# yellow-binary-tree/HeterSumGraph

Measured on AMD Instinct MI355X. Metric: graph-edges/sec through WSWGAT fwd+bwd, CNN/DM-shaped batch; 1/2/4/8 GPU, higher is better.
Workload: dtype f32; 1 GPU; cfg2: HSG WSWGAT stack W2S + 2x(S2W, W2S) fwd+bwd, train mode, 32 HSG docs/GPU x (N=35, W=600, k=36); gemm_operands=f32, bf16_rows=none, f32_rows=all, docs_per_gpu=32, graph_edges_per_gpu=159040, typed_edges_per_direction=40320, parallelism=dp1, dp_exchange=none (one rank), hip_graph=True

## Files before the change

### hetersumgraph_amd/_lib.py

```python
from __future__ import annotations

import ctypes
import os

import torch

_HERE = os.path.dirname(os.path.abspath(__file__))
LIB_PATH = os.environ.get("HSG_LIB_PATH") or os.path.join(_HERE, "libhsg.so")

HSG_EINVAL = 1001
HSG_TAU_TABLE = 0
HSG_TAU_PER_EDGE = 1

EXPORTS = ("hsg_gat_fwd", "hsg_gat_bwd_dst", "hsg_gat_bwd_blocks", "hsg_gat_bwd_src",
           "hsg_gat_bwd_src_blocks", "hsg_attn_src_logits", "hsg_attn_params_fwd", "hsg_attn_params_fwd_pair", "hsg_attn_params_fwd_pair_seed", "hsg_attn_params_finish_pair", "hsg_attn_params_bwd",
           "hsg_attn_params_bwd_workspace_floats", "hsg_version", "hsg_gemm_f32", "hsg_gemm_f32_mfma", "hsg_gemm_bf16", "hsg_gemm_workspace_floats", "hsg_gemm_auto_splits", "hsg_gemm_row_tiles", "hsg_ffn_colsums",
           "hsg_ln_bwd_blocks", "hsg_ln_fwd", "hsg_ln_bwd",
           "hsg_dropmask_words", "hsg_dropmask_scale", "hsg_dropmask", "hsg_hproj_fwd", "hsg_hproj_dx",
           "hsg_hproj_dw_chunks", "hsg_hproj_dw", "hsg_hproj_bwd", "hsg_rel_build_workspace_bytes", "hsg_rel_build",
           "hsg_cnn_taps", "hsg_cnn_gather", "hsg_cnn_pool", "hsg_cnn_pool_bwd",
           "hsg_ffn_small_supported", "hsg_ffn_small_fwd", "hsg_ffn_small_bwd_blocks", "hsg_ffn_small_bwd",
           "hsg_attn_params_stage", "hsg_attn_params_finish", "hsg_hproj_fwd_logits_supported",
           "hsg_hproj_fwd_logits", "hsg_wsplit_dims", "hsg_wsplit", "hsg_gemm_f32_psw", "hsg_dropmask_multi", "hsg_dropmask_multi_wt", "hsg_step_prologue", "hsg_gemm_f32_slabs", "hsg_slab_reduce",
           "hsg_hproj_wt", "hsg_hproj_fwd_t8_supported", "hsg_hproj_fwd_t8", "hsg_hproj_fwd_mf_supported", "hsg_hproj_fwd_mf", "hsg_kclock_arm",
           "hsg_kclock_pending", "hsg_seed_advance", "hsg_gat_bwd_dst_noh_supported", "hsg_gat_bwd_dst_noh",
           "hsg_gat_bwd_dst_g", "hsg_gemm_f32_psw_elug", "hsg_gemm_bf16_psw",
           "hsg_gemm_bf16_slabs", "hsg_gemm_dw_slabs", "hsg_gemm_dw_tiles", "hsg_gemm_psw_row_tiles", "hsg_gemm_psw_ln",
           "hsg_gat_bwd_src_g_supported", "hsg_gat_bwd_src_g", "hsg_gemm_psw_elug_rho", "hsg_ffn_small_bwd_gate",
           "hsg_gat_bwd_src_g_blocks", "hsg_gemm_bf16_psw_io", "hsg_gemm_bf16_psw_elug_rho_a16", "hsg_gemm_psw_elug_rho_gw", "hsg_ln_bwd_dy16",
           "hsg_gemm_dw_slabs_io", "hsg_ln_fwd_y16", "hsg_gat_bwd_src_g_io", "hsg_rel_work", "hsg_gat_fwd_ws_floats",
           "hsg_gat_fwd_ws", "hsg_gat_bwd_src_g_ws_floats", "hsg_gat_bwd_src_g_ws", "hsg_gat_fwd_ws16",
           "hsg_gemm_bf16_psw_elug_rho_x16", "hsg_ln_fwd_x16", "hsg_ln_bwd_x16")

HSG_EPI_STORE = 0
HSG_EPI_RELU_BWD = 1
HSG_EPI_ADD = 2
HSG_EPI_ADD_ELUG = 3
HSG_IO_A_BF16 = 1
HSG_IO_C_BF16 = 2
HSG_IO_AUX_BF16 = 4


class HsgRel(ctypes.Structure):

    _fields_ = [("n_src", ctypes.c_int32), ("n_dst", ctypes.c_int32), ("n_edges", ctypes.c_int32),
                ("indptr", ctypes.c_void_p), ("src", ctypes.c_void_p), ("tf", ctypes.c_void_p),
                ("phantom", ctypes.c_void_p), ("cindptr", ctypes.c_void_p),
                ("cdst", ctypes.c_void_p), ("cperm", ctypes.c_void_p),
                ("n_dwork", ctypes.c_int32), ("n_swork", ctypes.c_int32),
                ("dwork", ctypes.c_void_p), ("swork", ctypes.c_void_p)]


_lib = None

_P = ctypes.c_void_p
_I = ctypes.c_int
_F = ctypes.c_float
_RELP = ctypes.POINTER(HsgRel)

_SIGS = {
    "hsg_gat_fwd": [_RELP, _I, _I, _I, _F, _P, _P, _P, _P, _P, _P, _P, _P, _P],
    "hsg_gat_bwd_dst": [_RELP, _I, _I, _I, _I, _F, _P, _P, _P, _P, _P, _P, _P, _P, _P, _P, _P],
    "hsg_gat_bwd_blocks": [_RELP],
    "hsg_gat_bwd_src": [_RELP, _I, _I, _I, _F, _P, _P, _P, _P, _P, _P, _P, _P, _P, _P, _P, _P],
    "hsg_gat_bwd_src_blocks": [_RELP],
# ... 33 lines not shown
    "hsg_hproj_fwd_mf_supported": [_I, _I, _I],
    "hsg_hproj_fwd_mf": [_I, _I, _I, _P, _I, _P, _I, _I, _P, _F, _P, _I, _P, _P, _P],
    "hsg_hproj_dx": [_I, _I, _I, _I, _P, _I, _P, _P, _F, _P, _I, _I, _P],
    "hsg_hproj_dw_chunks": [_I, _I, _I, _I],
    "hsg_hproj_bwd": [_I, _I, _I, _I, _P, _I, _P, _P, _I, _P, _F, _P, _I, _I, _P, _P],
    "hsg_hproj_dw": [_I, _I, _I, _I, _P, _I, _P, _I, _P, _F, _P, _P, _I, _P],
    "hsg_rel_build_workspace_bytes": [_I, _I],
    "hsg_rel_build": [_F, _F, _I, _I] + [_P] * 17 + [ctypes.c_size_t, _P],
    "hsg_cnn_taps": [],
    "hsg_cnn_gather": [_I, _I, _I, _P, _P, _P, _P, ctypes.c_long, _P, _P],
    "hsg_cnn_pool": [_I, _I, _P, _P, _I, _P, _P, _P, _P],
    "hsg_cnn_pool_bwd": [_I, _P, _P, _P, _P, _P, _I, _P],
    "hsg_ln_fwd": [_I, _I, _P, _P, _P, _P, _F, _F, _P, ctypes.c_uint32, _P, _P, _P, _P],
    "hsg_ffn_small_supported": [_I, _I],
    "hsg_ffn_small_bwd_blocks": [_I],
    "hsg_ffn_small_bwd": [_I, _I, _I] + [_P] * 9 + [_F, _P, ctypes.c_uint32] + [_P] * 6,
    "hsg_ffn_small_bwd_gate": [_I, _I, _I] + [_P] * 9 + [_F, _P, ctypes.c_uint32] + [_P] * 9,
    "hsg_ffn_small_fwd": [_I, _I, _I, _P, _P, _P, _P, _P, _P, _P, _F, _F, _P, ctypes.c_uint32, _P, _P, _P, _P, _P,
                          _P],
    "hsg_ln_bwd": [_I, _I, _P, _P, _P, _P, _P, _P, _F, _P, ctypes.c_uint32, _P, _P, _P, _P],
    "hsg_wsplit_dims": [_I, _I, _P, _P],
    "hsg_dropmask_multi": [_I, _P, _P, _P, _P, _P, _P, _P, _P],
    "hsg_dropmask_multi_wt": [_I, _P, _P, _P, _P, _P, _P, _P, _I, _I, _I, _P, _P, _P],
    "hsg_step_prologue": [_I, _P, _P, _P, _P, _P, _P, _P, _I, _I, _I, _P, _P, _I, _P, _P, _P, _P, _P, _P, _P],
    "hsg_gemm_f32_slabs": [_I, _I, _I, _P, _I, _I, _P, _I, _I, _I, _P, _P],
    "hsg_gemm_bf16_slabs": [_I, _I, _I, _P, _I, _I, _P, _I, _I, _I, _P, _P],
    "hsg_gemm_dw_slabs": [_I, _P, _P, _I, _P, _P, _P, _P, _I, _I, _P, _P],
    "hsg_gemm_dw_tiles": [_I, _I],
    "hsg_gemm_psw_row_tiles": [_I, _I, _I, _I],
    "hsg_gemm_psw_ln": [_I, _I, _I, _P, _I, _P, _P, _P, _P, _P, _P, _F, _F, _P, ctypes.c_uint32, _P, _P, _P, _I, _P],
    "hsg_slab_reduce": [_I, _P, _P, _P, _P, _P, _P, _P, _P, _P, _P, _P],
    "hsg_wsplit": [_I, _P, _P, _P, _P, _P, _P, _P],
    "hsg_gemm_f32_psw": [_I, _I, _I, _P, _I, _P, _P, _I, _P, _P, _I, _I, _I, _P, _P],
    "hsg_gemm_f32_psw_elug": [_I, _I, _I, _P, _I, _P, _P, _I, _P, _P, _P, _P, _I, _I, _P],
    "hsg_gemm_bf16_psw": [_I, _I, _I, _P, _I, _P, _P, _I, _P, _P, _I, _I, _I, _P, _P],
    "hsg_gat_bwd_dst_g": [_RELP, _I, _I, _I, _F, _P, _P, _P, _P, _P, _P, _P, _P, _P],
    "hsg_gat_bwd_src_g_supported": [_RELP, _I, _I],
    "hsg_gat_bwd_src_g_blocks": [_RELP, _I, _I],
    "hsg_gat_bwd_src_g": [_RELP, _I, _I, _F, _P, _P, _P, _P, _P, _P, _I, _P, _P, _P, _P, _P, _P, _P],
    "hsg_gemm_psw_elug_rho": [_I, _I, _I, _P, _I, _P, _P, _I, _P, _P, _P, _P, _I, _P, _I, _I, _P],
    "hsg_gemm_bf16_psw_io": [_I, _I, _I, _P, _I, _P, _P, _I, _P, _P, _I, _I, _I, _P, _I, _P],
    "hsg_gemm_bf16_psw_elug_rho_a16": [_I, _I, _I, _P, _I, _P, _P, _I, _P, _P, _P, _P, _I, _P, _I, _I, _P],
    "hsg_gemm_psw_elug_rho_gw": [_I, _I, _I, _I, _I],
    "hsg_ln_bwd_dy16": [_I, _I, _P, _P, _I, _P, _P, _P, _P, _F, _P, ctypes.c_uint32, _P, _I, _P, _P, _P],
    "hsg_ln_fwd_y16": [_I, _I, _P, _P, _P, _P, _F, _F, _P, ctypes.c_uint32, _P, _P, _P, _P],
    "hsg_gat_bwd_src_g_io": [_RELP, _I, _I, _F, _P, _P, _P, _P, _P, _I, _P, _I, _P, _P, _P, _P, _P, _P, _P],
    "hsg_gemm_dw_slabs_io": [_I, _P, _P, _I, _P, _P, _P, _P, _P, _I, _P, _P],
    "hsg_rel_work": [_I, _P, _I, _I, _P, _I, _P, _P],
    "hsg_gat_fwd_ws_floats": [_RELP, _I, _I],
    "hsg_gat_fwd_ws": [_RELP, _I, _I, _I, _F, _P, _P, _P, _P, _P, _P, _P, _P, _P, _P],
    "hsg_gat_fwd_ws16": [_RELP, _I, _I, _I, _F, _P, _P, _P, _P, _P, _P, _P, _P, _P, _P, _I, _P],
    "hsg_gemm_bf16_psw_elug_rho_x16": [_I, _I, _I, _P, _I, _P, _P, _I, _P, _P, _I, _I, _P, _P, _I, _P, _I, _I, _P],
    "hsg_ln_fwd_x16": [_I, _I, _P, _P, _I, _P, _P, _F, _F, _P, ctypes.c_uint32, _P, _P, _P, _P],
    "hsg_ln_bwd_x16": [_I, _I, _P, _P, _P, _I, _P, _P, _P, _F, _P, ctypes.c_uint32, _P, _I, _P, _P, _P],
    "hsg_gat_bwd_src_g_ws_floats": [_RELP, _I, _I],
    "hsg_gat_bwd_src_g_ws": [_RELP, _I, _I, _F, _P, _P, _P, _P, _P, _I, _P, _I, _P, _P, _P, _P, _P, _P, _P, _P],
}
_RESTYPE = {"hsg_version": ctypes.c_char_p, "hsg_wsplit_dims": None, "hsg_gemm_workspace_floats": ctypes.c_size_t,
            "hsg_attn_params_bwd_workspace_floats": ctypes.c_size_t,
            "hsg_dropmask_scale": ctypes.c_float,
            "hsg_rel_build_workspace_bytes": ctypes.c_size_t, "hsg_gat_fwd_ws_floats": ctypes.c_size_t,
            "hsg_gat_bwd_src_g_ws_floats": ctypes.c_size_t}


def load():
    global _lib
# ... 108 lines not shown
```

### hetersumgraph_amd/csrc/hsg_gemm.hip

```cpp
#include <hip/hip_runtime.h>
#include <type_traits>
#include <stdint.h>
#include <stdlib.h>

#include <atomic>

#include "../../include/hsg.h"
#include "hsg_dev.h"
#include "hsg_wave.h"
#include "hsg_rng.h"
#include "hsg_wsplit.h"

namespace {

typedef float f32x16 __attribute__((ext_vector_type(16)));
typedef float f32x4 __attribute__((ext_vector_type(4)));
typedef __bf16 bf16x8 __attribute__((ext_vector_type(8)));

constexpr int kBK = 32;
constexpr int kPad = 4;

struct GemmArgs {
    int M, N, K;
    const float *A;
// ... 773 lines not shown
        bn = f32x4{0.f, 0.f, 0.f, 0.f};
        if (p.bias) bn = *reinterpret_cast<const f32x4 *>(p.bias + nc);
        if (p.epi != HSG_EPI_STORE) {
#pragma unroll
            for (int t = 0; t < STEPS; ++t) {
                const int m = min(row0 + min(t * RPS + rs, 31), p.M - 1);
                if constexpr (AUXBF) {
                    auxb[t] = *reinterpret_cast<const bf16x4v7 *>(
                        reinterpret_cast<const __bf16 *>(p.aux) + (size_t)m * p.ldaux + nc);
                } else {
                    aux[t] = *reinterpret_cast<const f32x4 *>(p.aux + (size_t)m * p.ldaux + nc);
                }
            }
        }
        if (p.epi == HSG_EPI_ADD_ELUG) {
#pragma unroll
            for (int t = 0; t < STEPS; ++t) {
                const int m = min(row0 + min(t * RPS + rs, 31), p.M - 1);
                const size_t o = (size_t)m * p.ldaux + nc;
                if constexpr (XBF) {
                    const bf16x4v7 xb = *reinterpret_cast<const bf16x4v7 *>(
                        reinterpret_cast<const __bf16 *>(p.aux2) + (size_t)m * p.ldx + nc);
                    ex[t] = f32x4{(float)xb[0], (float)xb[1], (float)xb[2], (float)xb[3]} -
                            *reinterpret_cast<const f32x4 *>(p.aux3 + o);
                } else {
                    ex[t] = *reinterpret_cast<const f32x4 *>(p.aux2 + o) - *reinterpret_cast<const f32x4 *>(p.aux3 + o);
                }
            }
        }
    }

    template <bool NS = false>
    __device__ __forceinline__ void finish(const float *wl, int row0, int col0, int lane, const GemmArgs &p,
                                           f32x4 &csum) {
        __builtin_amdgcn_s_waitcnt(0xc07f);
        __builtin_amdgcn_wave_barrier();
        const int q = lane % QS, rs = lane / QS;
        const int n = col0 + 4 * q;
        const bool qok = q < QPR && rs < RPS && n < p.N;
        const bool rho = p.epi == HSG_EPI_ADD_ELUG && p.rho;
        int slot[4] = {3, 3, 3, 3};
        if (rho) {
            const int hb = (n / GW * GW) / p.rho_d;
#pragma unroll
            for (int e = 0; e < 4; ++e) slot[e] = n + e < p.N ? (n + e) / p.rho_d - hb : 3;
        }
        csum = f32x4{0.f, 0.f, 0.f, 0.f};
#pragma unroll
        for (int t = 0; t < STEPS; ++t) {
            const int r = t * RPS + rs, m = row0 + r;
            const bool rok = r < 32 && m < p.M;
            float c[3] = {0.f, 0.f, 0.f};
            if (qok && rok) {
                f32x4 v = *reinterpret_cast<const f32x4 *>(&wl[r * LDW + 4 * q]);
                if (p.epi == HSG_EPI_RELU_BWD) {
                    if constexpr (AUXBF) {
#pragma unroll
                        for (int e = 0; e < 4; ++e) v[e] = (float)auxb[t][e] > 0.f ? v[e] : 0.f;
                    } else {
#pragma unroll
                        for (int e = 0; e < 4; ++e) v[e] = aux[t][e] > 0.f ? v[e] : 0.f;
                    }
                } else {
                    v += bn;
                    if (p.epi == HSG_EPI_ADD || p.epi == HSG_EPI_ADD_ELUG) v += aux[t];
                    if (p.relu) {
#pragma unroll
                        for (int e = 0; e < 4; ++e) v[e] = fmaxf(v[e], 0.f);
                    }
                }
                if constexpr (CBF) {
                    *reinterpret_cast<bf16x4v7 *>(reinterpret_cast<__bf16 *>(p.C) + (size_t)m * p.ldc + n) =
                        bf16x4v7{(__bf16)v[0], (__bf16)v[1], (__bf16)v[2], (__bf16)v[3]};
                } else if (!NS || v[0] == 1234.5f) {
                    *reinterpret_cast<f32x4 *>(p.C + (size_t)m * p.ldc + n) = v;
                }
                if (p.epi == HSG_EPI_ADD_ELUG) {
                    f32x4 g;
#pragma unroll
                    for (int e = 0; e < 4; ++e) g[e] = ex[t][e] > 0.f ? v[e] : v[e] * (ex[t][e] + 1.f);
                    if constexpr (GBF)
                        *reinterpret_cast<bf16x4v7 *>(reinterpret_cast<__bf16 *>(p.C2) + (size_t)m * p.ldaux + n) =
                            bf16x4v7{(__bf16)g[0], (__bf16)g[1], (__bf16)g[2], (__bf16)g[3]};
                    else
// ... 399 lines not shown
            }
        }
        __builtin_amdgcn_iglp_opt(0);
    }

    __syncthreads();
    float *wl = lds + wid * 32 * (BN + 4);
    const int c = lane & 15, rq = 4 * (lane >> 4);
#pragma unroll
    for (int i = 0; i < 2; ++i)
#pragma unroll
        for (int j = 0; j < TN; ++j)
#pragma unroll
            for (int e = 0; e < 4; ++e) wl[(16 * i + rq + e) * (BN + 4) + 16 * j + c] = acc[i][j][e];
    f32x4 cs;
    if (nt == 0) ep.load(p, m0 + wid * 32, n0, lane);
    ep.template finish<PM == 4>(wl, m0 + wid * 32, n0, lane, p, cs);
    if (p.colpart) epi_rows_colpart<BN>(lds, cs, wid, lane, ty, n0, p);
}

template <int BN, int S, int PM = 0, int OCC = 2, bool SA = false, int IO = 0>
int launch7(GemmArgs p, const __bf16 *planes, int Np, int Kp, hipStream_t st) {
    p.splits = 1;
    p.k_tiles_per_split = Kp / 32;
    if ((p.N + BN - 1) / BN * BN > Np) return HSG_EINVAL;
    if (!epi_rows_ok(p)) return HSG_EINVAL;
    const long g = (long)((p.N + BN - 1) / BN) * ((p.M + 127) / 128);
    if (SA && ((long)p.M * p.lda * 4 >= (1L << 32) || (long)3 * Np * Kp * 2 >= (1L << 32))) return HSG_EINVAL;
    hipLaunchKernelGGL((k_gemm7<BN, S, PM, OCC, SA, IO>), dim3((unsigned)g), dim3(256), 0, st, p, planes, Np, Kp);
    hipError_t e = hipGetLastError();
    return e == hipSuccess ? 0 : (int)e;
}

#ifdef HSG_DEV
constexpr int kG12BN = 64;
constexpr int kG12MaxKp = 320;

__host__ __device__ constexpr size_t g12_lds_bytes(int nt) {
    return (size_t)nt * 3 * kG12BN * 32 * 2 + (size_t)4 * 32 * (kG12BN + 4) * 4;
}

template <bool IGLP>
__global__ __launch_bounds__(256, 1) void k_gemm12(GemmArgs p, const __bf16 *__restrict__ planes, int Np, int Kp,
                                                   int tiles_n, int q) {
    constexpr int BN = kG12BN, TN = BN / 16, BPC = BN / 16, B_BF = BN * 32;
    extern __shared__ __attribute__((aligned(16))) float g12_lds[];
    const int nt = Kp / 32;
    __bf16 *sB = reinterpret_cast<__bf16 *>(g12_lds);
    const int lane = threadIdx.x & 63;
    const int wid = __builtin_amdgcn_readfirstlane(threadIdx.x >> 6);
    float *wl = g12_lds + nt * 3 * B_BF / 2 + wid * 32 * (BN + 4);
    const int xcd = blockIdx.x & 7, local = blockIdx.x >> 3;
    const int ct = local % tiles_n, sub = local / tiles_n;
    const int n0 = ct * BN;
    const int nbands = (p.M + 31) / 32;
    const int bb = xcd * nbands / 8, be = (xcd + 1) * nbands / 8;
    const int S = 4 * q, s = 4 * sub + wid;

    for (int pc = wid; pc < nt * 3 * BPC; pc += 4) {
        const int kt = pc / (3 * BPC), rem = pc % (3 * BPC);
        const int limb = rem / BPC, prow = (rem % BPC) * 16;
        const int r = prow + (lane >> 2);
        const int c = (lane & 3) ^ bswz16(r);
        const __bf16 *src = planes + ((size_t)(limb * Np + n0 + r) * Kp + kt * 32 + 8 * c);
        __builtin_amdgcn_global_load_lds((const __attribute__((address_space(1))) void *)src,
                                         (__attribute__((address_space(3))) void *)(sB + (kt * 3 + limb) * B_BF +
// ... 428 lines not shown
}

bool gemm11_on() {
    const char *e = HSG_DEV_ENV("HSG_GEMM11");
    return e && atoi(e) >= 1;
}

int plan11(int M, int N, int cus) {
    if (N > 512) return 0;
    const int BM = N > 320 ? 160 : 192, BN = N > 320 ? 256 : 160;
    const long tiles = (long)((M + BM - 1) / BM) * ((N + BN - 1) / BN);
    if (tiles > cus || 4 * tiles < 3L * cus) return 0;
    return N > 320 ? 1 : 2;
}

int device_cus() {
    static std::atomic<int> cached{-1};
    int c = cached.load(std::memory_order_relaxed);
    if (c < 0) {
        int dev = 0;
        c = 0;
        if (hipGetDevice(&dev) == hipSuccess && hipDeviceGetAttribute(&c, hipDeviceAttributeMultiprocessorCount, dev) != hipSuccess)
            c = 0;
        cached.store(c, std::memory_order_relaxed);
    }
    return c;
}

bool wide112_pays(int M, int N) {
    const int cus = device_cus() > 0 ? device_cus() : 256;
    const long slots = 2L * cus, mt = (M + 127) / 128;
    const long r112 = (mt * ((N + 111) / 112) + slots - 1) / slots, r64 = (mt * ((N + 63) / 64) + slots - 1) / slots;
    return r112 * 112 < r64 * 64;
}

template <int BM, int BN, int WGM, int WGN, int PM, int S = 2, int OCC = 1>
int launch11(GemmArgs p, const __bf16 *planes, int Np, int Kp, hipStream_t st) {
    p.splits = 1;
    p.k_tiles_per_split = Kp / 32;
    if ((p.N + BN - 1) / BN * BN > Np) return HSG_EINVAL;
    if (!epi_rows_ok(p)) return HSG_EINVAL;
    const long g = (long)((p.N + BN - 1) / BN) * ((p.M + BM - 1) / BM);
    hipLaunchKernelGGL((k_gemm11<BM, BN, WGM, WGN, PM, false, S, OCC>), dim3((unsigned)g), dim3(64 * WGM * WGN), 0, st, p, planes, Np,
                       Kp);
    hipError_t e = hipGetLastError();
    return e == hipSuccess ? 0 : (int)e;
}

int plan11ln(int M, int N, int cus) {
    if (N > 304 || N % 4) return 0;
    const long t96 = (M + 95) / 96, t128 = (M + 127) / 128;
    if (t96 <= cus && 5 * t96 >= 3L * cus) return 96;
    if (t128 <= cus && 5 * t128 >= 3L * cus) return 128;
    return 0;
}

template <int PM>
int try11ln(GemmArgs p, const __bf16 *planes, int Np, int Kp, hipStream_t st) {
    const int bm = plan11ln(p.M, p.N, device_cus());
    p.splits = 1;
    p.k_tiles_per_split = Kp / 32;
    if (!bm || 320 > Np) return HSG_EINVAL;
    const unsigned g = (unsigned)((p.M + bm - 1) / bm);
    if (bm == 96)
        hipLaunchKernelGGL((k_gemm11<96, 320, 2, 4, PM, true>), dim3(g), dim3(512), 0, st, p, planes, Np, Kp);
    else
// ... 556 lines not shown

int hsg_gemm_f32_mfma(int M, int N, int K, const float *A, int lda, int a_kcontig, const float *B, int ldb,
                      int b_kcontig, float *C, int ldc, const float *bias, const float *aux, int ldaux, int epi,
                      int relu, int splits, float *workspace, float *colsum_part, void *stream) {
    return gemm_impl(MODE_F32_MFMA, M, N, K, A, lda, a_kcontig, B, ldb, b_kcontig, C, ldc, bias, aux, ldaux, epi,
                     relu, splits, workspace, colsum_part, stream);
}

int hsg_gemm_bf16(int M, int N, int K, const float *A, int lda, int a_kcontig, const float *B, int ldb,
                  int b_kcontig, float *C, int ldc, const float *bias, const float *aux, int ldaux, int epi,
                  int relu, int splits, float *workspace, float *colsum_part, void *stream) {
    return gemm_impl(MODE_BF16, M, N, K, A, lda, a_kcontig, B, ldb, b_kcontig, C, ldc, bias, aux, ldaux, epi, relu,
                     splits, workspace, colsum_part, stream);
}

void hsg_wsplit_dims(int N, int K, int *Np, int *Kp) {
    *Np = (N + 127) / 128 * 128;
    *Kp = (K + 31) / 32 * 32;
}

int hsg_wsplit(int njobs, const float *const *W, const int *N, const int *K, const int *ldw, const int *trans,
               void *const *planes, void *stream) {
    if (njobs < 1 || njobs > 4) return HSG_EINVAL;
    HsgWSplitJobs j{};
    if (hsg_wsplit_setup(j, njobs, W, N, K, ldw, trans, planes)) return HSG_EINVAL;
    hipLaunchKernelGGL(k_wsplit, dim3(j.start[njobs]), dim3(256), 0, (hipStream_t)stream, j);
    hipError_t e = hipGetLastError();
    return e == hipSuccess ? 0 : (int)e;
}

int hsg_gemm_f32_psw(int M, int N, int K, const float *A, int lda, const void *planes, float *C, int ldc,
                     const float *bias, const float *aux, int ldaux, int epi, int relu, float *colsum_part,
                     void *stream) {
    if (M < 0 || N < 0 || K < 0 || !C || !planes || !A) return HSG_EINVAL;
    if (epi != HSG_EPI_STORE && epi != HSG_EPI_RELU_BWD && epi != HSG_EPI_ADD) return HSG_EINVAL;
    if (epi != HSG_EPI_STORE && !aux) return HSG_EINVAL;
    if ((lda & 3) || (K & 3) || (((uintptr_t)A) & 15) || (((uintptr_t)planes) & 15) || lda < K) return HSG_EINVAL;
    if (M == 0 || N == 0) return 0;
    int Np, Kp;
    hsg_wsplit_dims(N, K, &Np, &Kp);
    GemmArgs p{M, N, K, A, lda, nullptr, 0, C, ldc, bias, aux, ldaux, epi, relu, Kp / 32, nullptr, colsum_part, 1, 1};
    if (const char *x = HSG_DEV_ENV("HSG_GEMM_XCD")) p.xcd = atoi(x);
    const __bf16 *pl = reinterpret_cast<const __bf16 *>(planes);
    hipStream_t st = (hipStream_t)stream;
#ifdef HSG_DEV
    int plan = 27;
    if (const char *f = HSG_DEV_ENV("HSG_GEMM5")) plan = atoi(f);
    if (plan == 2) return launch5<128, 2>(p, pl, Np, Kp, st);
    if (plan == 3) return launch5<64, 3>(p, pl, Np, Kp, st);
    if (plan == 4) return launch5<128, 3>(p, pl, Np, Kp, st);
    if (plan == 5) return launch6<64>(p, pl, Np, Kp, st);
    if (plan == 6) return launch6<128>(p, pl, Np, Kp, st);
    if (plan == 7) return launch5<64, 2, 0>(p, pl, Np, Kp, st);
    if (plan == 8) return launch5<64, 2, 1>(p, pl, Np, Kp, st);
    if (plan == 24) return launch5<64, 2, 0, true>(p, pl, Np, Kp, st);
    if (plan == 25) return launch5<64, 2, 0, true, true>(p, pl, Np, Kp, st);
    if (plan == 26) return launch5<128, 2, 0, true, true>(p, pl, Np, Kp, st);
    if (plan == 28 && epi_rows_ok(p)) return launch7<64, 2, 1>(p, pl, Np, Kp, st);
    if (plan == 30 && epi_rows_ok(p)) return N <= 320 ? launch7<80, 2>(p, pl, Np, Kp, st) : launch7<128, 2>(p, pl, Np, Kp, st);
    if (plan == 34 && epi_rows_ok(p)) return launch7<64, 2, 4>(p, pl, Np, Kp, st);
    if (plan == 35 && epi_rows_ok(p)) return launch7<64, 2, 5>(p, pl, Np, Kp, st);
    if (plan == 36 && epi_rows_ok(p)) return launch7<64, 2, 6>(p, pl, Np, Kp, st);
    if (plan == 37 && epi_rows_ok(p)) return launch7<64, 2, 7>(p, pl, Np, Kp, st);
    if (plan == 38 && epi_rows_ok(p)) return launch7<64, 2, 8>(p, pl, Np, Kp, st);
    if (plan == 40 && epi_rows_ok(p)) return launch7<64, 2, 0, 2, true>(p, pl, Np, Kp, st);
    if (plan == 41 && epi_rows_ok(p))
        return N <= 320 ? launch7<80, 2, 0, 2, true>(p, pl, Np, Kp, st) : launch7<64, 2, 0, 2, true>(p, pl, Np, Kp, st);
    if (plan == 43 && epi_rows_ok(p))
        return N <= 320 && (N + 111) / 112 * 112 <= Np ? launch7<112, 2, 0, 2, true>(p, pl, Np, Kp, st)
                                                       : launch7<64, 2, 0, 2, true>(p, pl, Np, Kp, st);
    if (plan == 44 && epi_rows_ok(p)) return launch7<64, 2>(p, pl, Np, Kp, st);
    if (plan != 27) return launch5<64, 2>(p, pl, Np, Kp, st);
    if (gemm11_on()) {
        const int rc = try11<0>(p, pl, Np, Kp, st);
        if (rc != HSG_EINVAL || (colsum_part && atoi(HSG_DEV_ENV("HSG_GEMM11")) == 1 && plan11(M, N, device_cus())))
            return rc;
    }
#endif
#ifdef HSG_DEV
    if (plan12(M, N, K)) {
        const int rc = launch12(p, pl, Np, Kp, st);
        if (rc != HSG_EINVAL || colsum_part) return rc;
    }
#endif
    if (epi_rows_ok(p))
        return N <= 320 && (N + 111) / 112 * 112 <= Np && wide112_pays(M, N) ? launch7<112, 2>(p, pl, Np, Kp, st)
                                                                             : launch7<64, 2>(p, pl, Np, Kp, st);
    return launch5<64, 2, 0>(p, pl, Np, Kp, st);
}

extern "C++" {
template <int IO>
static int launch7io_narrow(GemmArgs p, const __bf16 *pl, int Np, int Kp, hipStream_t st) {
#ifdef HSG_DEV
    if (const char *e = HSG_DEV_ENV("HSG_GEMM7IO")) {
        const int v = atoi(e);
        if (v == 1) return launch7<128, 2, 2, 2, false, IO>(p, pl, Np, Kp, st);
        if (v == 3) return launch7<64, 2, 2, 3, false, IO>(p, pl, Np, Kp, st);
        if (v == 4) return launch7<64, 2, 2, 2, false, IO>(p, pl, Np, Kp, st);
    }
#endif
    return launch7<64, 3, 2, 3, false, IO>(p, pl, Np, Kp, st);
}
}

static int launch7io(GemmArgs p, const __bf16 *pl, int Np, int Kp, int io, hipStream_t st) {
    const bool wide = p.N > 320;
    switch (io) {
    case 0: return wide ? launch7<128, 2, 2>(p, pl, Np, Kp, st) : launch7<64, 2, 2>(p, pl, Np, Kp, st);
    case 1: return wide ? launch7<128, 2, 2, 2, false, 1>(p, pl, Np, Kp, st) : launch7io_narrow<1>(p, pl, Np, Kp, st);
    case 2: return wide ? launch7<128, 2, 2, 2, false, 2>(p, pl, Np, Kp, st) : launch7io_narrow<2>(p, pl, Np, Kp, st);
    case 7: return wide ? launch7<128, 2, 2, 2, false, 7>(p, pl, Np, Kp, st) : launch7io_narrow<7>(p, pl, Np, Kp, st);
    case 3: return wide ? launch7<128, 2, 2, 2, false, 3>(p, pl, Np, Kp, st) : launch7io_narrow<3>(p, pl, Np, Kp, st);
    case 9: return wide ? launch7<128, 2, 2, 2, false, 9>(p, pl, Np, Kp, st) : launch7io_narrow<9>(p, pl, Np, Kp, st);
    case 25: return wide ? launch7<128, 2, 2, 2, false, 25>(p, pl, Np, Kp, st) : launch7io_narrow<25>(p, pl, Np, Kp, st);
    default: return HSG_EINVAL;
    }
// ... 197 lines not shown
```

### hetersumgraph_amd/dense.py

```python
from __future__ import annotations

import contextlib
import ctypes

import torch

from . import _lib
from ._lib import HSG_EINVAL, HSG_EPI_ADD, HSG_EPI_RELU_BWD, HSG_EPI_STORE, check, load, ptr, stream_of


_GEMM_DTYPE = "f32"
_FNS = {"f32": "hsg_gemm_f32", "f32mfma": "hsg_gemm_f32_mfma", "bf16": "hsg_gemm_bf16"}


def set_gemm_dtype(dtype):
    global _GEMM_DTYPE
    if dtype not in _FNS:
        raise ValueError(f"gemm dtype must be one of {sorted(_FNS)}, not {dtype!r}")
    _GEMM_DTYPE = dtype


def get_gemm_dtype():
    return _GEMM_DTYPE

# ... 59 lines not shown
    return np_.value, kp.value


def split_weights(*specs, launch=True):
    lib = load()
    if not 1 <= len(specs) <= 4:
        raise ValueError("split_weights: 1..4 weights per launch")
    out, Ns, Ks, lds, trs, Ws, Ps = [], [], [], [], [], [], []
    for W, trans in specs:
        if not W.is_cuda or W.dtype != torch.float32 or W.dim() != 2 or W.stride(1) != 1:
            raise RuntimeError("split_weights: 2-D row-major fp32 ROCm tensors only")
        N, K = (W.shape[1], W.shape[0]) if trans else (W.shape[0], W.shape[1])
        Np, Kp = split_dims(N, K)
        planes = torch.empty(3 * Np * Kp, dtype=torch.bfloat16, device=W.device)
        out.append(SplitWeight(planes, N, K, W, bool(trans), "bf16" if _GEMM_DTYPE == "bf16" else "f32"))
        Ns.append(N); Ks.append(K); lds.append(W.stride(0)); trs.append(int(trans))
        Ws.append(W.data_ptr()); Ps.append(planes.data_ptr())
    n = len(specs)
    arr_i = ctypes.c_int * n
    arr_p = ctypes.c_void_p * n
    job = (n, arr_p(*Ws), arr_i(*Ns), arr_i(*Ks), arr_i(*lds), arr_i(*trs), arr_p(*Ps))
    if not launch:
        return out, job
    check(lib.hsg_wsplit(*job, stream_of(specs[0][0])), "hsg_wsplit")
    return out


def _io(A, out, aux):
    bf = torch.bfloat16
    return ((_lib.HSG_IO_A_BF16 if A.dtype == bf else 0) | (_lib.HSG_IO_C_BF16 if out.dtype == bf else 0)
            | (_lib.HSG_IO_AUX_BF16 if aux is not None and aux.dtype == bf else 0))


def gemm_psw(A, Bs, out=None, bias=None, relu=False, relu_mask=None, add=None, colsum_part=None):
    lib = load()
    if not A.is_cuda or A.dtype not in (torch.float32, torch.bfloat16):
        raise RuntimeError("hsg gemm: fp32 ROCm tensors only (no CPU fallback)")
    M, K = A.shape
    if K != Bs.K:
        raise ValueError(f"gemm_psw: inner dims {K} != {Bs.K}")
    N = Bs.N
    if out is None:
        out = A.new_empty(M, N, dtype=torch.float32)
    epi, aux = HSG_EPI_STORE, None
    if relu_mask is not None:
        epi, aux = HSG_EPI_RELU_BWD, relu_mask
    elif add is not None:
        epi, aux = HSG_EPI_ADD, add
    io = _io(A, out, aux)
    if io:
        if Bs.mode != "bf16":
            raise RuntimeError("gemm_psw: bf16 activations belong to the 'bf16' GEMM mode")
        check(lib.hsg_gemm_bf16_psw_io(M, N, K, ptr(A), _ld(A), ptr(Bs.planes), ptr(out), _ld(out), ptr(bias),
                                       ptr(aux), _ld(aux) if aux is not None else 0, epi, int(relu),
                                       ptr(colsum_part), io, stream_of(A)), "hsg_gemm_bf16_psw_io")
        return out
    if Bs.mode == "bf16":
        rc = lib.hsg_gemm_bf16_psw(M, N, K, ptr(A), _ld(A), ptr(Bs.planes), ptr(out), _ld(out), ptr(bias), ptr(aux),
                                   _ld(aux) if aux is not None else 0, epi, int(relu), ptr(colsum_part), stream_of(A))
        if rc == HSG_EINVAL and Bs.W is not None:
            if colsum_part is not None and colsum_part.shape[0] != row_tiles(M, N, K, 1):
                raise RuntimeError("gemm_psw: column partials sized for the split-weight kernel, which "
                                   "declined this call (alignment)")
            return gemm(A, Bs.W, b_t=not Bs.trans, out=out, bias=bias, relu=relu, relu_mask=relu_mask, add=add,
                        splits=1 if colsum_part is not None else 0, colsum_part=colsum_part, dtype="bf16")
        check(rc, "hsg_gemm_bf16_psw")
        return out
    check(lib.hsg_gemm_f32_psw(M, N, K, ptr(A), _ld(A), ptr(Bs.planes), ptr(out), _ld(out), ptr(bias), ptr(aux),
                               _ld(aux) if aux is not None else 0, epi, int(relu), ptr(colsum_part),
                               stream_of(A)), "hsg_gemm_f32_psw")
    return out


def gemm_psw_ln(A, Bs, bias, x, gamma, beta, eps, p_drop, seed_t, offset, y, out, mean, rstd):
    if _lib.path_option("HSG_FFN_LN_EPI", "0") != "1":
        return False
    lib = load()
    M, K = A.shape
    N = Bs.N
    if K != Bs.K or any(t.shape != (M, N) or not t.is_contiguous() for t in (x, y, out)):
        return False
    if any(t.dtype != torch.float32 for t in (A, x, y, out)):
        return False
    rc = lib.hsg_gemm_psw_ln(M, N, K, ptr(A), _ld(A), ptr(Bs.planes), ptr(bias), ptr(y), ptr(x), ptr(gamma),
                             ptr(beta), float(eps), float(p_drop), ptr(seed_t), offset, ptr(out), ptr(mean),
                             ptr(rstd), int(Bs.mode == "bf16"), stream_of(A))
    if rc == HSG_EINVAL:
        return False
    check(rc, "hsg_gemm_psw_ln")
    return True


def elug_rho_groups(Bs, M, head_dim):
    gw = load().hsg_gemm_psw_elug_rho_gw(M, Bs.N, Bs.K, int(head_dim), int(Bs.mode == "bf16"))
    return (Bs.N + gw - 1) // gw


def gemm_psw_elug(A, Bs, out, x, origin, G, rho=None, head_dim=0):
    lib = load()
    M, K = A.shape
    N = Bs.N
    x16 = x.dtype == torch.bfloat16
    ts = (out, origin, G) if x16 else (out, x, origin, G)
# ... 134 lines not shown
```

### include/hsg.h

```cpp
#ifndef HSG_H_
#define HSG_H_

#include <stddef.h>
#include <stdint.h>

#ifdef __cplusplus
extern "C" {
#endif

#define HSG_EINVAL 1001

typedef struct hsg_rel {
    int32_t n_src;
    int32_t n_dst;
    int32_t n_edges;
    const int32_t *indptr;
    const int32_t *src;
    const uint8_t *tf;
    const int32_t *phantom;
    const int32_t *cindptr;
    const int32_t *cdst;
    const int32_t *cperm;
    int32_t n_dwork;
    int32_t n_swork;
// ... 79 lines not shown
                          const float *da1_part, float *workspace, int accumulate, void *stream);
int hsg_attn_params_finish(int H, int D, int F, const float *workspace, const float *attn, const float *wf,
                           const float *bf, const float *T, float *dattn, float *dwf, float *dbf, float *dT,
                           int accumulate, void *stream);

int hsg_attn_params_finish_pair(int H0, int D0, const float *ws0, const float *attn0, const float *wf0,
                                const float *bf0, float *dattn0, float *dwf0, float *dbf0, float *dT0, int acc0,
                                int H1, int D1, const float *ws1, const float *attn1, const float *wf1,
                                const float *bf1, float *dattn1, float *dwf1, float *dbf1, float *dT1, int acc1,
                                int F, const float *T, void *stream);
size_t hsg_attn_params_bwd_workspace_floats(int H, int D);

#define HSG_EPI_STORE 0
#define HSG_EPI_RELU_BWD 1
#define HSG_EPI_ADD 2
#define HSG_EPI_ADD_ELUG 3
size_t hsg_gemm_workspace_floats(int M, int N, int K, int splits);
int hsg_gemm_auto_splits(int M, int N, int K);
int hsg_gemm_f32(int M, int N, int K, const float *A, int lda, int a_kcontig,
                 const float *B, int ldb, int b_kcontig, float *C, int ldc,
                 const float *bias, const float *aux, int ldaux, int epi, int relu,
                 int splits, float *workspace, float *colsum_part, void *stream);
int hsg_gemm_row_tiles(int M, int N, int K, int splits);
int hsg_gemm_f32_mfma(int M, int N, int K, const float *A, int lda, int a_kcontig,
                      const float *B, int ldb, int b_kcontig, float *C, int ldc,
                      const float *bias, const float *aux, int ldaux, int epi, int relu,
                      int splits, float *workspace, float *colsum_part, void *stream);
void hsg_wsplit_dims(int N, int K, int *Np, int *Kp);
int hsg_wsplit(int njobs, const float *const *W, const int *N, const int *K, const int *ldw,
               const int *trans, void *const *planes, void *stream);
int hsg_gemm_f32_psw(int M, int N, int K, const float *A, int lda, const void *planes,
                     float *C, int ldc, const float *bias, const float *aux, int ldaux,
                     int epi, int relu, float *colsum_part, void *stream);
int hsg_gemm_f32_psw_elug(int M, int N, int K, const float *A, int lda, const void *planes, float *C, int ldc,
                          const float *aux, const float *x, const float *origin, float *G, int ld, int bf16,
                          void *stream);
int hsg_gemm_psw_elug_rho(int M, int N, int K, const float *A, int lda, const void *planes, float *C, int ldc,
                          const float *aux, const float *x, const float *origin, float *G, int ld, float *rho,
                          int head_dim, int bf16, void *stream);
int hsg_gemm_psw_elug_rho_gw(int M, int N, int K, int head_dim, int bf16);
int hsg_gemm_bf16_psw(int M, int N, int K, const float *A, int lda, const void *planes, float *C, int ldc,
                      const float *bias, const float *aux, int ldaux, int epi, int relu, float *colsum_part,
                      void *stream);
#define HSG_IO_A_BF16 1
#define HSG_IO_C_BF16 2
#define HSG_IO_AUX_BF16 4
int hsg_gemm_bf16_psw_io(int M, int N, int K, const void *A, int lda, const void *planes, void *C, int ldc,
                         const float *bias, const void *aux, int ldaux, int epi, int relu, float *colsum_part,
                         int io, void *stream);
int hsg_gemm_bf16_psw_elug_rho_a16(int M, int N, int K, const void *A, int lda, const void *planes, float *C,
                                   int ldc, const float *aux, const float *x, const float *origin, void *G, int ld,
                                   float *rho, int head_dim, int g_bf16, void *stream);
int hsg_gemm_bf16_psw_elug_rho_x16(int M, int N, int K, const void *A, int lda, const void *planes, float *C,
                                   int ldc, const float *aux, const void *x, int ldx, int x_bf16, const float *origin,
                                   void *G, int ld, float *rho, int head_dim, int g_bf16, void *stream);
int hsg_gemm_f32_slabs(int M, int N, int K, const float *A, int lda, int a_kcontig,
                       const float *B, int ldb, int b_kcontig, int splits, float *workspace,
                       void *stream);
int hsg_gemm_bf16_slabs(int M, int N, int K, const float *A, int lda, int a_kcontig,
                        const float *B, int ldb, int b_kcontig, int splits, float *workspace,
                        void *stream);
int hsg_gemm_psw_ln(int M, int N, int K, const float *A, int lda, const void *planes, const float *bias, float *y,
                    const float *x, const float *gamma, const float *beta, float eps, float p_drop, const int64_t *seed,
                    uint32_t offset, float *out, float *mean, float *rstd, int bf16, void *stream);
int hsg_gemm_psw_row_tiles(int M, int N, int K, int bf16);
int hsg_gemm_dw_slabs(int njobs, const int *M, const int *N, int K, const float *const *A, const int *lda,
// ... 114 lines not shown
```

Before: 140.7 million graph-edges/s.

## Add taller-tile 3-limb bf16 MFMA GEMM kernel for wide fp32 pre-split-weight GEMMs

```diff
diff --git a/hetersumgraph_amd/_lib.py b/hetersumgraph_amd/_lib.py
--- a/hetersumgraph_amd/_lib.py
+++ b/hetersumgraph_amd/_lib.py
@@ -30,7 +30,7 @@
            "hsg_gat_bwd_src_g_blocks", "hsg_gemm_bf16_psw_io", "hsg_gemm_bf16_psw_elug_rho_a16", "hsg_gemm_psw_elug_rho_gw", "hsg_ln_bwd_dy16",
            "hsg_gemm_dw_slabs_io", "hsg_ln_fwd_y16", "hsg_gat_bwd_src_g_io", "hsg_rel_work", "hsg_gat_fwd_ws_floats",
            "hsg_gat_fwd_ws", "hsg_gat_bwd_src_g_ws_floats", "hsg_gat_bwd_src_g_ws", "hsg_gat_fwd_ws16",
-           "hsg_gemm_bf16_psw_elug_rho_x16", "hsg_ln_fwd_x16", "hsg_ln_bwd_x16")
+           "hsg_gemm_bf16_psw_elug_rho_x16", "hsg_ln_fwd_x16", "hsg_ln_bwd_x16", "hsg_gemm_f32_psw_plan", "hsg_gemm_f32_psw_route")
 
 HSG_EPI_STORE = 0
 HSG_EPI_RELU_BWD = 1
@@ -130,6 +130,8 @@
     "hsg_slab_reduce": [_I, _P, _P, _P, _P, _P, _P, _P, _P, _P, _P, _P],
     "hsg_wsplit": [_I, _P, _P, _P, _P, _P, _P, _P],
     "hsg_gemm_f32_psw": [_I, _I, _I, _P, _I, _P, _P, _I, _P, _P, _I, _I, _I, _P, _P],
+    "hsg_gemm_f32_psw_route": [_I, _I, _I],
+    "hsg_gemm_f32_psw_plan": [_I, _I, _I, _P, _I, _P, _P, _I, _P, _P, _I, _I, _I, _P, _I, _P],
     "hsg_gemm_f32_psw_elug": [_I, _I, _I, _P, _I, _P, _P, _I, _P, _P, _P, _P, _I, _I, _P],
     "hsg_gemm_bf16_psw": [_I, _I, _I, _P, _I, _P, _P, _I, _P, _P, _I, _I, _I, _P, _P],
     "hsg_gat_bwd_dst_g": [_RELP, _I, _I, _I, _F, _P, _P, _P, _P, _P, _P, _P, _P, _P],
diff --git a/hetersumgraph_amd/csrc/hsg_gemm.hip b/hetersumgraph_amd/csrc/hsg_gemm.hip
--- a/hetersumgraph_amd/csrc/hsg_gemm.hip
+++ b/hetersumgraph_amd/csrc/hsg_gemm.hip
@@ -829,7 +829,7 @@
 
     template <bool NS = false>
     __device__ __forceinline__ void finish(const float *wl, int row0, int col0, int lane, const GemmArgs &p,
-                                           f32x4 &csum) {
+                                           f32x4 &csum, int rmax = 32) {
         __builtin_amdgcn_s_waitcnt(0xc07f);
         __builtin_amdgcn_wave_barrier();
         const int q = lane % QS, rs = lane / QS;
@@ -846,7 +846,7 @@
 #pragma unroll
         for (int t = 0; t < STEPS; ++t) {
             const int r = t * RPS + rs, m = row0 + r;
-            const bool rok = r < 32 && m < p.M;
+            const bool rok = r < rmax && m < p.M;
             float c[3] = {0.f, 0.f, 0.f};
             if (qok && rok) {
                 f32x4 v = *reinterpret_cast<const f32x4 *>(&wl[r * LDW + 4 * q]);
@@ -1312,6 +1312,169 @@
     return e == hipSuccess ? 0 : (int)e;
 }
 
+template <int TM>
+__global__ __launch_bounds__(256, 2) void k_gemm13(GemmArgs p, const __bf16 *__restrict__ planes, int Np, int Kp) {
+    constexpr int BM = 32 * TM, BN = 128, WM = 16 * TM, NB = (TM + 1) / 2;
+    constexpr int A_FL = BM * 32;
+    constexpr int B_BF = BN * 32;
+    constexpr int STAGE_FL = A_FL + 3 * B_BF / 2;
+    constexpr int EPI_FL = 4 * 32 * 68;
+    constexpr int RED_FL = TM % 2 == 0 ? (BM / 32) * 4 * BN : 0;
+    __shared__ __attribute__((aligned(16))) float lds[STAGE_FL > EPI_FL + RED_FL ? STAGE_FL : EPI_FL + RED_FL];
+    const int lane = threadIdx.x & 63;
+    const int wid = __builtin_amdgcn_readfirstlane(threadIdx.x >> 6);
+    const int wr = wid >> 1, wc = wid & 1;
+    const int tiles_n = (p.N + BN - 1) / BN, tiles_m = (p.M + BM - 1) / BM;
+    const int total = tiles_n * tiles_m;
+    const int lt = p.xcd ? xcd_tile(blockIdx.x, total) : (int)blockIdx.x;
+    const int tx = lt % tiles_n, ty = lt / tiles_n;
+    const int m0 = ty * BM, n0 = tx * BN;
+    const int nt = Kp / 32;
+    __builtin_assume(p.epi != HSG_EPI_ADD_ELUG);
+
+    f32x4v7 acc[TM][4];
+#pragma unroll
+    for (int i = 0; i < TM; ++i)
+#pragma unroll
+        for (int j = 0; j < 4; ++j) acc[i][j] = f32x4v7{0.f, 0.f, 0.f, 0.f};
+
+    auto issue_a = [&](int it, int pc) {
+        const int piece = pc * 4 + wid;
+        const int r = piece * 8 + (lane >> 3);
+        const int k = it * 32 + 4 * ((lane & 7) ^ swz16(r));
+        const float *src = k < p.K ? p.A + (size_t)min(m0 + r, p.M - 1) * p.lda + k : g_zero16;
+        __builtin_amdgcn_global_load_lds((const __attribute__((address_space(1))) void *)src,
+                                         (__attribute__((address_space(3))) void *)(lds + piece * 256), 16, 0, 0);
+    };
+    auto issue_b = [&](int it, int pc) {
+        __bf16 *sb = reinterpret_cast<__bf16 *>(lds + A_FL);
+        const int piece = pc * 4 + wid;
+        const int limb = piece / 8, prow = (piece % 8) * 16;
+        const int r = prow + (lane >> 2);
+        const int c = (lane & 3) ^ bswz16(r);
+        const __bf16 *src = planes + ((size_t)(limb * Np + n0 + r) * Kp + it * 32 + 8 * c);
+        __builtin_amdgcn_global_load_lds((const __attribute__((address_space(1))) void *)src,
+                                         (__attribute__((address_space(3))) void *)(sb + limb * B_BF + prow * 32),
+                                         16, 0, 0);
+    };
+    if (nt > 0) {
+#pragma unroll
+        for (int pc = 0; pc < TM; ++pc) issue_a(0, pc);
+#pragma unroll
+        for (int pc = 0; pc < 6; ++pc) issue_b(0, pc);
+    }
+    const int li = lane & 15, kb = lane >> 4;
+    const __bf16 *sb = reinterpret_cast<const __bf16 *>(lds + A_FL);
+    for (int it = 0; it < nt; ++it) {
+        wait_vmcnt<0>();
+        __builtin_amdgcn_s_barrier();
+        asm volatile("" ::: "memory");
+        f32x4 ax[TM], ay[TM];
+        bf16x8 b[4][3];
+#pragma unroll
+        for (int i = 0; i < TM; ++i) {
+            const int r = wr * WM + 16 * i + li, sw = swz16(r);
+            ax[i] = *reinterpret_cast<const f32x4 *>(&lds[r * 32 + 4 * ((2 * kb) ^ sw)]);
+            ay[i] = *reinterpret_cast<const f32x4 *>(&lds[r * 32 + 4 * ((2 * kb + 1) ^ sw)]);
+        }
+#pragma unroll
+        for (int j = 0; j < 4; ++j) {
+            const int r = wc * 64 + 16 * j + li;
+            const int off = r * 32 + 8 * (kb ^ bswz16(r));
+#pragma unroll
+            for (int l = 0; l < 3; ++l) b[j][l] = *reinterpret_cast<const bf16x8 *>(&sb[l * B_BF + off]);
+        }
+        asm volatile("s_waitcnt lgkmcnt(0)" ::: "memory");
+        __builtin_amdgcn_s_barrier();
+        asm volatile("" ::: "memory");
+        const bool more = it + 1 < nt;
+#pragma unroll
+        for (int i = 0; i < TM; ++i) {
+            bf16x8 a0, a1, a2;
+            if (more) {
+                issue_a(it + 1, i);
+                issue_b(it + 1, i);
+                if (i == TM - 1)
+                    for (int pc = TM; pc < 6; ++pc) issue_b(it + 1, pc);
+            }
+            split_rne8(ax[i], ay[i], a0, a1, a2);
+#pragma unroll
+            for (int j = 0; j < 4; ++j) acc[i][j] = __builtin_amdgcn_mfma_f32_16x16x32_bf16(a2, b[j][0], acc[i][j], 0, 0, 0);
+#pragma unroll
+            for (int j = 0; j < 4; ++j) acc[i][j] = __builtin_amdgcn_mfma_f32_16x16x32_bf16(a1, b[j][1], acc[i][j], 0, 0, 0);
+#pragma unroll
+            for (int j = 0; j < 4; ++j) acc[i][j] = __builtin_amdgcn_mfma_f32_16x16x32_bf16(a0, b[j][2], acc[i][j], 0, 0, 0);
+#pragma unroll
+            for (int j = 0; j < 4; ++j) acc[i][j] = __builtin_amdgcn_mfma_f32_16x16x32_bf16(a1, b[j][0], acc[i][j], 0, 0, 0);
+#pragma unroll
+            for (int j = 0; j < 4; ++j) acc[i][j] = __builtin_amdgcn_mfma_f32_16x16x32_bf16(a0, b[j][1], acc[i][j], 0, 0, 0);
+#pragma unroll
+            for (int j = 0; j < 4; ++j) acc[i][j] = __builtin_amdgcn_mfma_f32_16x16x32_bf16(a0, b[j][0], acc[i][j], 0, 0, 0);
+        }
+    }
+
+    __syncthreads();
+    float *wl = lds + wid * 32 * 68;
+    const int c = lane & 15, rq = 4 * (lane >> 4);
+    const int col0 = n0 + wc * 64;
+    EpiRows<64> eps[NB];
+    eps[0].load(p, m0 + wr * WM, col0, lane);
+#pragma unroll
+    for (int bd = 0; bd < NB; ++bd) {
+        const int row0 = m0 + wr * WM + 32 * bd;
+        const int rows = WM - 32 * bd < 32 ? WM - 32 * bd : 32;
+        if (bd + 1 < NB) eps[bd + 1].load(p, row0 + 32, col0, lane);
+#pragma unroll
+        for (int i = 0; i < 2; ++i)
+#pragma unroll
+            for (int j = 0; j < 4; ++j)
+#pragma unroll
+                for (int e = 0; e < 4; ++e)
+                    if (2 * bd + i < TM) wl[(16 * i + rq + e) * 68 + 16 * j + c] = acc[2 * bd + i < TM ? 2 * bd + i : 0][j][e];
+        f32x4 cs;
+        eps[bd].finish(wl, row0, col0, lane, p, cs, rows);
+        if constexpr (TM % 2 == 0) {
+            if (p.colpart)
+                *reinterpret_cast<f32x4 *>(&lds[EPI_FL + ((wr * NB + bd) * 4 + (lane >> 4)) * BN + wc * 64 +
+                                                4 * (lane & 15)]) = cs;
+        }
+        __builtin_amdgcn_wave_barrier();
+    }
+    if constexpr (TM % 2 == 0) {
+        if (p.colpart) {
+            const float *red = lds + EPI_FL;
+            __syncthreads();
+            const int rows64 = (p.M + 63) / 64;
+            for (int cc = threadIdx.x; cc < (BM / 64) * BN; cc += 256) {
+                const int s = cc / BN, col = cc % BN, n = n0 + col, slab = ty * (BM / 64) + s;
+                float v = 0.f;
+                for (int w = 2 * s; w < 2 * s + 2; ++w)
+                    for (int r = 0; r < 4; ++r) v += red[(w * 4 + r) * BN + col];
+                if (n < p.N && slab < rows64) p.colpart[(size_t)slab * p.N + n] = v;
+            }
+        }
+    }
+}
+
+template <int TM>
+int launch13(GemmArgs p, const __bf16 *planes, int Np, int Kp, hipStream_t st) {
+    constexpr int BM = 32 * TM;
+    p.splits = 1;
+    p.k_tiles_per_split = Kp / 32;
+    if ((p.N + 127) / 128 * 128 > Np) return HSG_EINVAL;
+    if (!epi_rows_ok(p)) return HSG_EINVAL;
+    if (p.colpart && BM % 64) return HSG_EINVAL;
+    const long g = (long)((p.N + 127) / 128) * ((p.M + BM - 1) / BM);
+    hipLaunchKernelGGL((k_gemm13<TM>), dim3((unsigned)g), dim3(256), 0, st, p, planes, Np, Kp);
+    hipError_t e = hipGetLastError();
+    return e == hipSuccess ? 0 : (int)e;
+}
+
+int gemm13_bm(const GemmArgs &p) { return p.colpart ? 192 : 160; }
+int launch13(GemmArgs p, const __bf16 *planes, int Np, int Kp, hipStream_t st) {
+    return p.colpart ? launch13<6>(p, planes, Np, Kp, st) : launch13<5>(p, planes, Np, Kp, st);
+}
+
 #ifdef HSG_DEV
 constexpr int kG12BN = 64;
 constexpr int kG12MaxKp = 320;
@@ -1806,6 +1969,15 @@
     const long slots = 2L * cus, mt = (M + 127) / 128;
     const long r112 = (mt * ((N + 111) / 112) + slots - 1) / slots, r64 = (mt * ((N + 63) / 64) + slots - 1) / slots;
     return r112 * 112 < r64 * 64;
+}
+
+bool gemm13_pays(int M, int N, int bm) {
+    if (N <= 320) return false;
+    const int cus = device_cus() > 0 ? device_cus() : 256;
+    const long slots = 2L * cus;
+    const long r13 = (((M + bm - 1) / bm) * (long)((N + 127) / 128) + slots - 1) / slots;
+    const long r7 = (((M + 127) / 128) * (long)((N + 63) / 64) + slots - 1) / slots;
+    return r13 * bm * 128 * 9 < r7 * 128 * 64 * 10;
 }
 
 template <int BM, int BN, int WGM, int WGN, int PM, int S = 2, int OCC = 1>
@@ -2428,6 +2600,18 @@
 int hsg_gemm_f32_psw(int M, int N, int K, const float *A, int lda, const void *planes, float *C, int ldc,
                      const float *bias, const float *aux, int ldaux, int epi, int relu, float *colsum_part,
                      void *stream) {
+    return hsg_gemm_f32_psw_plan(M, N, K, A, lda, planes, C, ldc, bias, aux, ldaux, epi, relu, colsum_part, 0, stream);
+}
+
+int hsg_gemm_f32_psw_route(int M, int N, int K) {
+    (void)K;
+    return gemm13_pays(M, N, 160) ? 13 : 7;
+}
+
+int hsg_gemm_f32_psw_plan(int M, int N, int K, const float *A, int lda, const void *planes, float *C, int ldc,
+                          const float *bias, const float *aux, int ldaux, int epi, int relu, float *colsum_part,
+                          int sel, void *stream) {
+    if (sel != 0 && sel != 7 && sel != 13) return HSG_EINVAL;
     if (M < 0 || N < 0 || K < 0 || !C || !planes || !A) return HSG_EINVAL;
     if (epi != HSG_EPI_STORE && epi != HSG_EPI_RELU_BWD && epi != HSG_EPI_ADD) return HSG_EINVAL;
     if (epi != HSG_EPI_STORE && !aux) return HSG_EINVAL;
@@ -2439,6 +2623,8 @@
     if (const char *x = HSG_DEV_ENV("HSG_GEMM_XCD")) p.xcd = atoi(x);
     const __bf16 *pl = reinterpret_cast<const __bf16 *>(planes);
     hipStream_t st = (hipStream_t)stream;
+    if (sel == 7) return epi_rows_ok(p) ? launch7<64, 2>(p, pl, Np, Kp, st) : HSG_EINVAL;
+    if (sel == 13) return launch13(p, pl, Np, Kp, st);
 #ifdef HSG_DEV
     int plan = 27;
     if (const char *f = HSG_DEV_ENV("HSG_GEMM5")) plan = atoi(f);
@@ -2479,6 +2665,7 @@
         if (rc != HSG_EINVAL || colsum_part) return rc;
     }
 #endif
+    if (epi_rows_ok(p) && gemm13_pays(M, N, gemm13_bm(p))) return launch13(p, pl, Np, Kp, st);
     if (epi_rows_ok(p))
         return N <= 320 && (N + 111) / 112 * 112 <= Np && wide112_pays(M, N) ? launch7<112, 2>(p, pl, Np, Kp, st)
                                                                              : launch7<64, 2>(p, pl, Np, Kp, st);
diff --git a/hetersumgraph_amd/dense.py b/hetersumgraph_amd/dense.py
--- a/hetersumgraph_amd/dense.py
+++ b/hetersumgraph_amd/dense.py
@@ -115,7 +115,7 @@
             | (_lib.HSG_IO_AUX_BF16 if aux is not None and aux.dtype == bf else 0))
 
 
-def gemm_psw(A, Bs, out=None, bias=None, relu=False, relu_mask=None, add=None, colsum_part=None):
+def gemm_psw(A, Bs, out=None, bias=None, relu=False, relu_mask=None, add=None, colsum_part=None, plan=0):
     lib = load()
     if not A.is_cuda or A.dtype not in (torch.float32, torch.bfloat16):
         raise RuntimeError("hsg gemm: fp32 ROCm tensors only (no CPU fallback)")
@@ -131,6 +131,8 @@
     elif add is not None:
         epi, aux = HSG_EPI_ADD, add
     io = _io(A, out, aux)
+    if plan and (io or Bs.mode == "bf16"):
+        raise ValueError("gemm_psw: plan selects among the fp32 mode's kernels only")
     if io:
         if Bs.mode != "bf16":
             raise RuntimeError("gemm_psw: bf16 activations belong to the 'bf16' GEMM mode")
@@ -149,9 +151,9 @@
                         splits=1 if colsum_part is not None else 0, colsum_part=colsum_part, dtype="bf16")
         check(rc, "hsg_gemm_bf16_psw")
         return out
-    check(lib.hsg_gemm_f32_psw(M, N, K, ptr(A), _ld(A), ptr(Bs.planes), ptr(out), _ld(out), ptr(bias), ptr(aux),
-                               _ld(aux) if aux is not None else 0, epi, int(relu), ptr(colsum_part),
-                               stream_of(A)), "hsg_gemm_f32_psw")
+    check(lib.hsg_gemm_f32_psw_plan(M, N, K, ptr(A), _ld(A), ptr(Bs.planes), ptr(out), _ld(out), ptr(bias), ptr(aux),
+                                    _ld(aux) if aux is not None else 0, epi, int(relu), ptr(colsum_part),
+                                    int(plan), stream_of(A)), "hsg_gemm_f32_psw_plan")
     return out
 
 
diff --git a/include/hsg.h b/include/hsg.h
--- a/include/hsg.h
+++ b/include/hsg.h
@@ -135,6 +135,10 @@
 int hsg_gemm_f32_psw(int M, int N, int K, const float *A, int lda, const void *planes,
                      float *C, int ldc, const float *bias, const float *aux, int ldaux,
                      int epi, int relu, float *colsum_part, void *stream);
+int hsg_gemm_f32_psw_plan(int M, int N, int K, const float *A, int lda, const void *planes,
+                          float *C, int ldc, const float *bias, const float *aux, int ldaux,
+                          int epi, int relu, float *colsum_part, int plan, void *stream);
+int hsg_gemm_f32_psw_route(int M, int N, int K);
 int hsg_gemm_f32_psw_elug(int M, int N, int K, const float *A, int lda, const void *planes, float *C, int ldc,
                           const float *aux, const float *x, const float *origin, float *G, int ld, int bf16,
                           void *stream);
```

New measurement: 151.5 million graph-edges/s, median of 6. 1.08x the previous value.
